# eora-ai/torchok

Measured on AMD Instinct MI355X. Metric: images/sec (node) ResNet-50 224px bs256/GPU; step p50 ms, higher is better.
Workload: dtype bf16

## Files before the change

torchok_amd/csrc/gemm256.hip:

```cpp
#include "conv_common.h"
#include <stdlib.h>

namespace {

typedef __attribute__((address_space(3))) void lds_void;
typedef __attribute__((address_space(3))) char lds_char;

constexpr int GT = 256;
constexpr int GK = 64;
constexpr int TILE_B = GT * GK * 2;
constexpr int STAGE_B = 2 * TILE_B;
constexpr int NBLK = STAGE_B / 1024;
constexpr int NI = NBLK / 8;

__device__ __forceinline__ u32x4 lds_read16(uint32_t addr) {
  u32x4 v;
  asm volatile("ds_read_b128 %0, %1" : "=v"(v) : "v"(addr));
  return v;
}
__device__ __forceinline__ float row16_sum_f(float v) {
  v += __builtin_bit_cast(float, __builtin_amdgcn_update_dpp(0, __builtin_bit_cast(int, v), 0x128, 0xF, 0xF, false));
  v += __builtin_bit_cast(float, __builtin_amdgcn_update_dpp(0, __builtin_bit_cast(int, v), 0x124, 0xF, 0xF, false));
  v += __builtin_bit_cast(float, __builtin_amdgcn_update_dpp(0, __builtin_bit_cast(int, v), 0x122, 0xF, 0xF, false));
  v += __builtin_bit_cast(float, __builtin_amdgcn_update_dpp(0, __builtin_bit_cast(int, v), 0x121, 0xF, 0xF, false));
  return v;
}

template <int MODE>
__global__ __launch_bounds__(512, 1) void gemm256_kernel(ConvArgs a) {
  extern __shared__ __attribute__((aligned(16))) char smem[];
  const uint32_t lds_base = (uint32_t)(size_t)(lds_char*)smem;
  const int tid = threadIdx.x;
  const int lane = tid & 63;
  const int wave = __builtin_amdgcn_readfirstlane(tid >> 6);
  const int r = lane & 15, g = lane >> 4;
  const int wn = wave & 1, wm = wave >> 1;

  const int ntiles = a.gridM * a.gridN;
  const int KD = a.Ktot;
  const int KT = (KD + GK - 1) / GK;

  const __amdgpu_buffer_rsrc_t xsrd = __builtin_amdgcn_make_buffer_rsrc((void*)a.x, 0, a.x_bytes, 0x00020000);
  const __amdgpu_buffer_rsrc_t wsrd = __builtin_amdgcn_make_buffer_rsrc((void*)a.w, 0, a.w_bytes, 0x00020000);

  uint32_t voff[NI];
  int kq[NI];
#pragma unroll
  for (int j = 0; j < NI; ++j) {
    const int row = ((j * 8 + wave) & 31) * 8 + (lane >> 3);
    kq[j] = ((lane & 7) ^ ((row & 3) | (((row >> 3) & 1) << 2))) * 8;
  }
  auto setup = [&](int id, int& m0, int& n0) {
    const int mt = id / a.gridN, nt = id - mt * a.gridN;
    m0 = mt * GT;
    n0 = nt * GT;
#pragma unroll
    for (int j = 0; j < NI; ++j) {
      const int bid = j * 8 + wave;
      const int row = (bid & 31) * 8 + (lane >> 3);
      const bool isw = bid < 32;
      const int grow = (isw ? n0 : m0) + row;
      const bool ok = grow < (isw ? a.K : a.M);
      voff[j] = ok ? (uint32_t)(((long long)grow * KD + kq[j]) * 2) : 0xFFFFFFF0u;
    }
  };
  auto issue = [&](int kt, int buf, bool live) {
#pragma unroll
    for (int j = 0; j < NI; ++j) {
      const int bid = j * 8 + wave;
      uint32_t off = (live && voff[j] != 0xFFFFFFF0u && kt * GK + kq[j] < KD) ? voff[j] + (uint32_t)(kt * (GK * 2)) : 0xFFFFFFF0u;
      asm volatile("" : "+v"(off));
      lds_void* dst = (lds_void*)(smem + buf * STAGE_B + bid * 1024);
      if (bid < 32) __builtin_amdgcn_raw_ptr_buffer_load_lds(wsrd, dst, 16, off, 0, 0, 0);
      else __builtin_amdgcn_raw_ptr_buffer_load_lds(xsrd, dst, 16, off, 0, 0, 0);
    }
  };

  const uint32_t swz = (uint32_t)((r & 3) | (((r >> 2) & 1) << 2));
  const uint32_t swx = (uint32_t)((r & 3) | (((r >> 3) & 1) << 2));
  const uint32_t a_lane = (uint32_t)((wn * 128 + 8 * (r >> 2) + (r & 3)) * 128);
  const uint32_t b_lane = (uint32_t)(TILE_B + (wm * 64 + r) * 128);
  uint32_t a_ch[2], b_ch[2];
#pragma unroll
  for (int kk = 0; kk < 2; ++kk) {
    a_ch[kk] = (((uint32_t)(4 * kk + g)) ^ swz) << 4;
    b_ch[kk] = (((uint32_t)(4 * kk + g)) ^ swx) << 4;
  }

  int tile = tok_xcd_remap(blockIdx.x, gridDim.x);
  int m0, n0;
  setup(tile, m0, n0);
  int base = 0;
  issue(0, base, tile < ntiles);
  while (tile < ntiles) {
  f32x4 acc[4][2][4];
#pragma unroll
  for (int p = 0; p < 4; ++p)
#pragma unroll
    for (int b = 0; b < 2; ++b)
#pragma unroll
      for (int mb = 0; mb < 4; ++mb) acc[p][b][mb] = (f32x4){0.f, 0.f, 0.f, 0.f};
  for (int kt = 0; kt < KT; ++kt) {
    const int buf = (base + kt) & 1;
    asm volatile("s_waitcnt vmcnt(0)" ::: "memory");
    __builtin_amdgcn_s_barrier();
    issue(kt + 1, buf ^ 1, kt + 1 < KT);
    const uint32_t sb = lds_base + (uint32_t)(buf * STAGE_B);
#pragma unroll
    for (int kk = 0; kk < 2; ++kk) {
      u32x4 af[4][2], bfr[4];
#pragma unroll
      for (int mb = 0; mb < 4; ++mb) bfr[mb] = lds_read16(sb + b_lane + (uint32_t)(mb * 16 * 128) + b_ch[kk]);
#pragma unroll
      for (int p = 0; p < 4; ++p)
#pragma unroll
        for (int b = 0; b < 2; ++b) af[p][b] = lds_read16(sb + a_lane + (uint32_t)((32 * p + 4 * b) * 128) + a_ch[kk]);
      asm volatile("s_waitcnt lgkmcnt(0)" ::: "memory");
      __builtin_amdgcn_sched_barrier(0);
#pragma unroll
      for (int p = 0; p < 4; ++p)
#pragma unroll
        for (int b = 0; b < 2; ++b)
#pragma unroll
          for (int mb = 0; mb < 4; ++mb)
            acc[p][b][mb] = __builtin_amdgcn_mfma_f32_16x16x32_bf16(__builtin_bit_cast(bf16x8, af[p][b]),
                                                                    __builtin_bit_cast(bf16x8, bfr[mb]), acc[p][b][mb], 0, 0, 0);
    }
  }
  const int cm0 = m0, cn0 = n0, cmt = m0 / GT;
  const int next = tile + gridDim.x;
  base = (base + KT) & 1;
  if (next < ntiles) {
    setup(next, m0, n0);
    issue(0, base, true);
  }

  float s1[4][8], s2[4][8];
  if constexpr (MODE >= 1 && MODE <= 3) {
#pragma unroll
    for (int p = 0; p < 4; ++p)
#pragma unroll
      for (int e = 0; e < 8; ++e) { s1[p][e] = 0.f; s2[p][e] = 0.f; }
  }
#pragma unroll
  for (int p = 0; p < 4; ++p) {
    const int n8 = cn0 + wn * 128 + 32 * p + 8 * g;
    const bool nok = n8 + 8 <= a.K;
    float bv[8];
#pragma unroll
    for (int e = 0; e < 8; ++e) bv[e] = (a.bias != nullptr && nok) ? a.bias[n8 + e] : 0.f;
#pragma unroll
    for (int mb = 0; mb < 4; ++mb) {
      const int pix = cm0 + wm * 64 + 16 * mb + r;
      if (pix < a.M && nok) {
        const size_t off = (size_t)pix * a.K + n8;
        float v[8];
#pragma unroll
        for (int e = 0; e < 8; ++e) v[e] = acc[p][e >> 2][mb][e & 3] + bv[e];
        if (a.accumulate) {
          const bf16x8 old = ldg16(a.y + off);
#pragma unroll
          for (int e = 0; e < 8; ++e) v[e] += bf2f(old[e]);
        }
        bf16x8 o;
#pragma unroll
        for (int e = 0; e < 8; ++e) o[e] = f2bf(v[e]);
        if constexpr (MODE == 3) {
          const unsigned bits = (unsigned)a.bn_mask[off >> 3];
#pragma unroll
          for (int e = 0; e < 8; ++e) {
            if (!((bits >> e) & 1u)) o[e] = (bf16)0.f;
            s1[p][e] += bf2f(o[e]);
          }
        }
        stg16(a.y + off, o);
        if constexpr (MODE == 1) {
#pragma unroll
          for (int e = 0; e < 8; ++e) {
            const float q = bf2f(o[e]);
            s1[p][e] += q;
            s2[p][e] = fmaf(q, q, s2[p][e]);
          }
        }
        if constexpr (MODE == 2) {
          const bf16x8 yv = ldg16(a.bn_y + off);
          const unsigned bits = a.bn_mask != nullptr ? (unsigned)a.bn_mask[off >> 3] : 0xffu;
#pragma unroll
          for (int e = 0; e < 8; ++e) {
            const float dz = ((bits >> e) & 1u) ? bf2f(o[e]) : 0.f;
            s1[p][e] += dz;
            s2[p][e] = fmaf(dz, bf2f(yv[e]), s2[p][e]);
          }
        }
      }
    }
  }
  if constexpr (MODE >= 1 && MODE <= 3) {
    float* red = reinterpret_cast<float*>(smem + 2 * STAGE_B);
#pragma unroll
    for (int p = 0; p < 4; ++p)
#pragma unroll
      for (int e = 0; e < 8; ++e) {
        const float t1 = row16_sum_f(s1[p][e]), t2 = row16_sum_f(s2[p][e]);
        if (r == 15) {
          const int nl = wn * 128 + 32 * p + 8 * g + e;
          red[(0 * 4 + wm) * GT + nl] = t1;
          red[(1 * 4 + wm) * GT + nl] = t2;
        }
      }
    asm volatile("s_waitcnt lgkmcnt(0)" ::: "memory");
    __builtin_amdgcn_s_barrier();
    const int which = tid >> 8, c = tid & 255;
    const float t = red[(which * 4 + 0) * GT + c] + red[(which * 4 + 1) * GT + c] + red[(which * 4 + 2) * GT + c] +
                    red[(which * 4 + 3) * GT + c];
    const int n = cn0 + c;
    if (n < a.K) a.stats[((size_t)which * a.stat_rows + cmt) * a.K + n] = t;
    if (cmt == a.gridM - 1 && n < a.K)
      for (int rr = a.gridM; rr < a.stat_rows; ++rr) a.stats[((size_t)which * a.stat_rows + rr) * a.K + n] = 0.f;
    asm volatile("s_waitcnt lgkmcnt(0)" ::: "memory");
    __builtin_amdgcn_s_barrier();
  }
  tile = next;
  }
  asm volatile("s_waitcnt vmcnt(0) lgkmcnt(0)" ::: "memory");
}

int g256_flag() {
  static const int v = [] { const char* e = getenv("TOK_GEMM256"); return (int)(e ? atoi(e) : 1); }();
  return v;
}
int g256_min_k() {
  static const int v = [] { const char* e = getenv("TOK_GEMM256_MIN_K"); return (int)(e ? atoi(e) : 256); }();
  return v;
}
int g256_min_tiles() {
  static const int v = [] { const char* e = getenv("TOK_GEMM256_MIN_TILES"); return (int)(e ? atoi(e) : 128); }();
  return v;
}

}

bool gemm256_modes(const ConvArgs& a) {
  if (a.ep_scale != nullptr || a.sub != nullptr) return false;
  if (a.mask_store && (a.bn_mask == nullptr || a.stats == nullptr)) return false;
  if (a.y2 != nullptr || a.act_x != nullptr) return false;
  return true;
}
bool gemm256_serves(const ConvArgs& a) { return gemm256_geometry(a) && gemm256_modes(a); }

bool gemm256_geometry(const ConvArgs& a) {
  const int flag = g256_flag();
  if (!flag) return false;
  if (!(a.R == 1 && a.S == 1 && a.stride == 1 && a.pad == 0 && a.C != 4)) return false;
  if (a.Ktot % 8 != 0 || a.K % 8 != 0 || a.Ktot <= GK) return false;
  if (flag >= 3) return true;
  if (a.K < 192 || a.M < 4096) return false;
  const long long tiles = (long long)tok_cdiv(a.M, GT) * tok_cdiv(a.K, GT);
  const int nt = tok_cdiv(a.K, GT);
  if ((long long)nt * GT * 3 > (long long)a.K * 4) return false;
  if (tiles < g256_min_tiles()) return false;
  if (flag >= 2) return a.Ktot >= g256_min_k();
  return a.Ktot >= 384;
}

int gemm256_rows(const ConvArgs& a) { return (tok_cdiv(a.M, GT) + 7) / 8 * 8; }

void gemm256_tiles(const ConvArgs& a, int* gridM, int* gridN) { *gridM = tok_cdiv(a.M, GT); *gridN = tok_cdiv(a.K, GT); }
int gemm256_grid(int gridM, int gridN) { return gridM * gridN < 256 ? gridM * gridN : 256; }

int gemm256_launch(ConvArgs& a, hipStream_t st) {
  constexpr int smem = 2 * STAGE_B + 2 * 4 * GT * 4;
  const int grid = a.grid;
  if (a.mask_store) tok_launch_lds<&gemm256_kernel<3>>(smem, dim3(grid), dim3(512), smem, st, a);
  else if (a.stats == nullptr) tok_launch_lds<&gemm256_kernel<0>>(smem, dim3(grid), dim3(512), smem, st, a);
  else if (a.bn_y == nullptr) tok_launch_lds<&gemm256_kernel<1>>(smem, dim3(grid), dim3(512), smem, st, a);
  else tok_launch_lds<&gemm256_kernel<2>>(smem, dim3(grid), dim3(512), smem, st, a);
  return 0;
}
```

Baseline: 14500.

## Split A/B tile loads into staggered half-stages with ping-pong wave groups

Restructures the 256x256 GEMM main loop so weight and activation tiles are loaded separately, each issued at a different half of the k-step, and keeps a deeper in-flight window (vmcnt(8)) in place of a full drain before each barrier. The two halves of the workgroup are offset by one barrier to ping-pong between LDS reads and MFMA, and MFMA phases run at raised priority. Loads for the next output tile continue seamlessly across tile boundaries. The epilogue vectorizes bias loads and batches the global loads for residual, mask and BN inputs ahead of the stores. This adds more barriers and more complex buffer-reuse logic, which risks races on the LDS buffers.

```diff
diff --git a/torchok_amd/csrc/gemm256.hip b/torchok_amd/csrc/gemm256.hip
--- a/torchok_amd/csrc/gemm256.hip
+++ b/torchok_amd/csrc/gemm256.hip
@@ -50,12 +50,13 @@
     const int row = ((j * 8 + wave) & 31) * 8 + (lane >> 3);
     kq[j] = ((lane & 7) ^ ((row & 3) | (((row >> 3) & 1) << 2))) * 8;
   }
-  auto setup = [&](int id, int& m0, int& n0) {
+  auto is_wb = [](int j) { return j == 1 || j == 3; };
+  auto setup = [&](int id, bool wb) {
     const int mt = id / a.gridN, nt = id - mt * a.gridN;
-    m0 = mt * GT;
-    n0 = nt * GT;
+    const int m0 = mt * GT, n0 = nt * GT;
 #pragma unroll
     for (int j = 0; j < NI; ++j) {
+      if (is_wb(j) != wb) continue;
       const int bid = j * 8 + wave;
       const int row = (bid & 31) * 8 + (lane >> 3);
       const bool isw = bid < 32;
@@ -64,9 +65,10 @@
       voff[j] = ok ? (uint32_t)(((long long)grow * KD + kq[j]) * 2) : 0xFFFFFFF0u;
     }
   };
-  auto issue = [&](int kt, int buf, bool live) {
+  auto issue = [&](bool wb, int kt, int buf, bool live) {
 #pragma unroll
     for (int j = 0; j < NI; ++j) {
+      if (is_wb(j) != wb) continue;
       const int bid = j * 8 + wave;
       uint32_t off = (live && voff[j] != 0xFFFFFFF0u && kt * GK + kq[j] < KD) ? voff[j] + (uint32_t)(kt * (GK * 2)) : 0xFFFFFFF0u;
       asm volatile("" : "+v"(off));
@@ -88,11 +90,25 @@
   }
 
   int tile = tok_xcd_remap(blockIdx.x, gridDim.x);
-  int m0, n0;
-  setup(tile, m0, n0);
-  int base = 0;
-  issue(0, base, tile < ntiles);
+  int atile = tile, akt = 0, btile = tile, bkt = 0;
+  auto adv = [&](bool wb, int& t, int& k) {
+    if (++k == KT) {
+      k = 0;
+      t += gridDim.x;
+      setup(t, wb);
+    }
+  };
+  setup(tile, false);
+  setup(tile, true);
+  int par = 0;
+  const int half = wave >> 2;
+  issue(false, akt, 0, atile < ntiles); adv(false, atile, akt);
+  issue(true, bkt, 0, btile < ntiles);  adv(true, btile, bkt);
+  issue(false, akt, 1, atile < ntiles); adv(false, atile, akt);
+  asm volatile("s_waitcnt vmcnt(8)" ::: "memory");
+  __builtin_amdgcn_s_barrier();
   while (tile < ntiles) {
+  const int m0 = (tile / a.gridN) * GT, n0 = (tile - (tile / a.gridN) * a.gridN) * GT;
   f32x4 acc[4][2][4];
 #pragma unroll
   for (int p = 0; p < 4; ++p)
@@ -100,40 +116,56 @@
     for (int b = 0; b < 2; ++b)
 #pragma unroll
       for (int mb = 0; mb < 4; ++mb) acc[p][b][mb] = (f32x4){0.f, 0.f, 0.f, 0.f};
+  if (half == 1) __builtin_amdgcn_s_barrier();
   for (int kt = 0; kt < KT; ++kt) {
-    const int buf = (base + kt) & 1;
-    asm volatile("s_waitcnt vmcnt(0)" ::: "memory");
-    __builtin_amdgcn_s_barrier();
-    issue(kt + 1, buf ^ 1, kt + 1 < KT);
-    const uint32_t sb = lds_base + (uint32_t)(buf * STAGE_B);
-#pragma unroll
-    for (int kk = 0; kk < 2; ++kk) {
-      u32x4 af[4][2], bfr[4];
-#pragma unroll
-      for (int mb = 0; mb < 4; ++mb) bfr[mb] = lds_read16(sb + b_lane + (uint32_t)(mb * 16 * 128) + b_ch[kk]);
-#pragma unroll
-      for (int p = 0; p < 4; ++p)
-#pragma unroll
-        for (int b = 0; b < 2; ++b) af[p][b] = lds_read16(sb + a_lane + (uint32_t)((32 * p + 4 * b) * 128) + a_ch[kk]);
-      asm volatile("s_waitcnt lgkmcnt(0)" ::: "memory");
+    const uint32_t sb = lds_base + (uint32_t)(par * STAGE_B);
+    u32x4 af[2][2][2], bfr[2][4];
+#pragma unroll
+    for (int h = 0; h < 2; ++h) {
+      if (h == 0) {
+#pragma unroll
+        for (int kk = 0; kk < 2; ++kk)
+#pragma unroll
+          for (int mb = 0; mb < 4; ++mb) bfr[kk][mb] = lds_read16(sb + b_lane + (uint32_t)(mb * 16 * 128) + b_ch[kk]);
+      }
+#pragma unroll
+      for (int kk = 0; kk < 2; ++kk)
+#pragma unroll
+        for (int pp = 0; pp < 2; ++pp)
+#pragma unroll
+          for (int b = 0; b < 2; ++b)
+            af[kk][pp][b] = lds_read16(sb + a_lane + (uint32_t)((32 * (2 * h + pp) + 4 * b) * 128) + a_ch[kk]);
+      if (h == 0) {
+        issue(true, bkt, par ^ 1, btile < ntiles);
+        adv(true, btile, bkt);
+      } else {
+        issue(false, akt, par, atile < ntiles);
+        adv(false, atile, akt);
+      }
+      asm volatile("s_waitcnt vmcnt(8) lgkmcnt(0)" ::: "memory");
+      __builtin_amdgcn_s_barrier();
       __builtin_amdgcn_sched_barrier(0);
-#pragma unroll
-      for (int p = 0; p < 4; ++p)
-#pragma unroll
-        for (int b = 0; b < 2; ++b)
-#pragma unroll
-          for (int mb = 0; mb < 4; ++mb)
-            acc[p][b][mb] = __builtin_amdgcn_mfma_f32_16x16x32_bf16(__builtin_bit_cast(bf16x8, af[p][b]),
-                                                                    __builtin_bit_cast(bf16x8, bfr[mb]), acc[p][b][mb], 0, 0, 0);
-    }
-  }
+      __builtin_amdgcn_s_setprio(1);
+#pragma unroll
+      for (int kk = 0; kk < 2; ++kk)
+#pragma unroll
+        for (int pp = 0; pp < 2; ++pp)
+#pragma unroll
+          for (int b = 0; b < 2; ++b)
+#pragma unroll
+            for (int mb = 0; mb < 4; ++mb)
+              acc[2 * h + pp][b][mb] = __builtin_amdgcn_mfma_f32_16x16x32_bf16(__builtin_bit_cast(bf16x8, af[kk][pp][b]),
+                                                                               __builtin_bit_cast(bf16x8, bfr[kk][mb]),
+                                                                               acc[2 * h + pp][b][mb], 0, 0, 0);
+      __builtin_amdgcn_s_setprio(0);
+      __builtin_amdgcn_sched_barrier(0);
+      __builtin_amdgcn_s_barrier();
+    }
+    par ^= 1;
+  }
+  if (half == 0) __builtin_amdgcn_s_barrier();
   const int cm0 = m0, cn0 = n0, cmt = m0 / GT;
   const int next = tile + gridDim.x;
-  base = (base + KT) & 1;
-  if (next < ntiles) {
-    setup(next, m0, n0);
-    issue(0, base, true);
-  }
 
   float s1[4][8], s2[4][8];
   if constexpr (MODE >= 1 && MODE <= 3) {
@@ -146,52 +178,84 @@
   for (int p = 0; p < 4; ++p) {
     const int n8 = cn0 + wn * 128 + 32 * p + 8 * g;
     const bool nok = n8 + 8 <= a.K;
-    float bv[8];
-#pragma unroll
-    for (int e = 0; e < 8; ++e) bv[e] = (a.bias != nullptr && nok) ? a.bias[n8 + e] : 0.f;
-#pragma unroll
-    for (int mb = 0; mb < 4; ++mb) {
-      const int pix = cm0 + wm * 64 + 16 * mb + r;
-      if (pix < a.M && nok) {
+    float bv[8] = {0.f, 0.f, 0.f, 0.f, 0.f, 0.f, 0.f, 0.f};
+    if (a.bias != nullptr) {
+      const float4* bp = reinterpret_cast<const float4*>(a.bias + (nok ? n8 : 0));
+      const float4 b0 = bp[0], b1 = bp[1];
+      bv[0] = nok ? b0.x : 0.f; bv[1] = nok ? b0.y : 0.f; bv[2] = nok ? b0.z : 0.f; bv[3] = nok ? b0.w : 0.f;
+      bv[4] = nok ? b1.x : 0.f; bv[5] = nok ? b1.y : 0.f; bv[6] = nok ? b1.z : 0.f; bv[7] = nok ? b1.w : 0.f;
+    }
+#pragma unroll
+    for (int mb = 0; mb < 4; ++mb)
+#pragma unroll
+      for (int e = 0; e < 8; ++e) acc[p][e >> 2][mb][e & 3] += bv[e];
+  }
+#pragma unroll
+  for (int p = 0; p < 4; ++p) {
+    const int n8 = cn0 + wn * 128 + 32 * p + 8 * g;
+    const bool nok = n8 + 8 <= a.K;
+    constexpr int GRP = MODE == 0 ? 4 : 2;
+#pragma unroll
+    for (int m0b = 0; m0b < 4; m0b += GRP) {
+      bf16x8 old[GRP], yv[GRP], o[GRP];
+      unsigned bits[GRP];
+#pragma unroll
+      for (int i = 0; i < GRP; ++i) {
+        const int pix = cm0 + wm * 64 + 16 * (m0b + i) + r;
         const size_t off = (size_t)pix * a.K + n8;
-        float v[8];
-#pragma unroll
-        for (int e = 0; e < 8; ++e) v[e] = acc[p][e >> 2][mb][e & 3] + bv[e];
-        if (a.accumulate) {
-          const bf16x8 old = ldg16(a.y + off);
-#pragma unroll
-          for (int e = 0; e < 8; ++e) v[e] += bf2f(old[e]);
+        bits[i] = 0xffu;
+        if (pix < a.M && nok) {
+          if (a.accumulate) old[i] = ldg16(a.y + off);
+          if constexpr (MODE == 2) {
+            yv[i] = ldg16(a.bn_y + off);
+            if (a.bn_mask != nullptr) bits[i] = (unsigned)a.bn_mask[off >> 3];
+          }
+          if constexpr (MODE == 3) bits[i] = (unsigned)a.bn_mask[off >> 3];
         }
-        bf16x8 o;
-#pragma unroll
-        for (int e = 0; e < 8; ++e) o[e] = f2bf(v[e]);
-        if constexpr (MODE == 3) {
-          const unsigned bits = (unsigned)a.bn_mask[off >> 3];
-#pragma unroll
-          for (int e = 0; e < 8; ++e) {
-            if (!((bits >> e) & 1u)) o[e] = (bf16)0.f;
-            s1[p][e] += bf2f(o[e]);
+      }
+#pragma unroll
+      for (int i = 0; i < GRP; ++i) {
+        const int mb = m0b + i;
+        const int pix = cm0 + wm * 64 + 16 * mb + r;
+        if (pix < a.M && nok) {
+          float v[8];
+#pragma unroll
+          for (int e = 0; e < 8; ++e) v[e] = acc[p][e >> 2][mb][e & 3];
+          if (a.accumulate) {
+#pragma unroll
+            for (int e = 0; e < 8; ++e) v[e] += bf2f(old[i][e]);
+          }
+#pragma unroll
+          for (int e = 0; e < 8; ++e) o[i][e] = f2bf(v[e]);
+          if constexpr (MODE == 3) {
+#pragma unroll
+            for (int e = 0; e < 8; ++e) {
+              if (!((bits[i] >> e) & 1u)) o[i][e] = (bf16)0.f;
+              s1[p][e] += bf2f(o[i][e]);
+            }
+          }
+          if constexpr (MODE == 1) {
+#pragma unroll
+            for (int e = 0; e < 8; ++e) {
+              const float q = bf2f(o[i][e]);
+              s1[p][e] += q;
+              s2[p][e] = fmaf(q, q, s2[p][e]);
+            }
+          }
+          if constexpr (MODE == 2) {
+#pragma unroll
+            for (int e = 0; e < 8; ++e) {
+              const float dz = ((bits[i] >> e) & 1u) ? bf2f(o[i][e]) : 0.f;
+              s1[p][e] += dz;
+              s2[p][e] = fmaf(dz, bf2f(yv[i][e]), s2[p][e]);
+            }
           }
         }
-        stg16(a.y + off, o);
-        if constexpr (MODE == 1) {
-#pragma unroll
-          for (int e = 0; e < 8; ++e) {
-            const float q = bf2f(o[e]);
-            s1[p][e] += q;
-            s2[p][e] = fmaf(q, q, s2[p][e]);
-          }
-        }
-        if constexpr (MODE == 2) {
-          const bf16x8 yv = ldg16(a.bn_y + off);
-          const unsigned bits = a.bn_mask != nullptr ? (unsigned)a.bn_mask[off >> 3] : 0xffu;
-#pragma unroll
-          for (int e = 0; e < 8; ++e) {
-            const float dz = ((bits >> e) & 1u) ? bf2f(o[e]) : 0.f;
-            s1[p][e] += dz;
-            s2[p][e] = fmaf(dz, bf2f(yv[e]), s2[p][e]);
-          }
-        }
+      }
+#pragma unroll
+      for (int i = 0; i < GRP; ++i) {
+        const int pix = cm0 + wm * 64 + 16 * (m0b + i) + r;
+        if (pix < a.M && nok) stg16(a.y + (size_t)pix * a.K + n8, o[i]);
       }
     }
   }
```

After: 14530 (median of 2 runs). Within noise of the previous version (+0.2%).
